# limuhit/360-Image-Compression

Measured on AMD Instinct MI355X. Metric: ERP Mpixels/s enc+dec @512x1024 model-idx 3; bitstream bit-exact vs ref, higher is better.
Workload: dtype f32; 1 GPU; 192/GPU synthetic 512x1024 ERPs, model-idx 3 --ssim seed, latent+importance bitstreams, entropy enc+dec; streams=3, masks=smooth

## Files before the change

### 360-image-compression_amd/csrc/cconv144_kernels.hip

```cpp
#include "common.h"
#include "conv_plan.h"
#include "cconv_tree.h"

#define I144_THREADS 512

template <int C, int HIDDEN>
struct ITerms {
    static constexpr int NIDX = 25 * C;
    static constexpr bool causal(int tap) { return tap / 5 + tap % 5 <= 3 + HIDDEN; }
    static constexpr int nterms(int l) {
        int n = 0;
        for (int i = l; i < NIDX; i += 128) n += causal(i % 25) ? 1 : 0;
        return n;
    }
    static constexpr int term(int l, int t) {
        int n = 0;
        for (int i = l; i < NIDX; i += 128)
            if (causal(i % 25)) { if (n == t) return i; ++n; }
        return -1;
    }
    static constexpr int nquads(int l) { return (nterms(l) + 3) / 4; }
    static constexpr int qbase(int l) {
        int s = 0;
        for (int j = 0; j < l; ++j) s += nquads(j);
        return s;
    }
    static constexpr int NQ = qbase(128);
    static constexpr int nblocks(int c) { int s = 0; for (int a = 0; a < 16; ++a) s += nquads(c + 8 * a); return s; }
    static constexpr int blk_a(int c, int b) { int a = 0; while (b >= nquads(c + 8 * a)) { b -= nquads(c + 8 * a); ++a; } return a; }
    static constexpr int blk_q(int c, int b) { int a = 0; while (b >= nquads(c + 8 * a)) { b -= nquads(c + 8 * a); ++a; } return b; }
    static constexpr int ngroups() { int m = 0; for (int c = 0; c < 8; ++c) { const int g = (nblocks(c) + 3) / 4; m = g > m ? g : m; } return m; }
    static constexpr int NG = ngroups();
};

static inline bool conv144_ok(const lic360_conv_plan *p) {
    return p->ksz == 5 && p->ngroup == 1 && p->C == 144 && p->nout >= 1 && p->nout <= 144 && p->constrain == 6;
}
template <int HIDDEN> static int i144_nq() { return ITerms<144, HIDDEN>::NQ; }
static int conv144_nq(const lic360_conv_plan *p) { (void)p; return i144_nq<1>(); }
static int conv144_otiles(const lic360_conv_plan *p) { return (p->nout + 15) / 16; }

__global__ void k_conv144_pack(const float *__restrict__ weight, const int *__restrict__ src, const int *__restrict__ qmap, float *__restrict__ packed,
                               int nout, int C, int NG, long total) {
    for (long e = (long)blockIdx.x * blockDim.x + threadIdx.x; e < total; e += (long)gridDim.x * blockDim.x) {
        const int jw = (int)(e & 3), l = (int)((e >> 2) & 63), i = l & 15, k = l >> 4;
        const long t = e >> 8;
        const int g = (int)(t % NG), c = (int)((t / NG) & 7), ot = (int)(t / (8 * NG)), o = ot * 16 + i;
        const int Q = qmap[(c * NG + g) * 4 + jw];
        const int s = Q >= 0 ? src[Q * 4 + k] : -1;
        packed[e] = (s >= 0 && o < nout) ? weight[(long)o * C * 25 + s] : 0.0f;
    }
}
template <int HIDDEN>
static void i144_fill_src(int *src, int *qmap) {
    using T = ITerms<144, HIDDEN>;
    int Q = 0;
    for (int l = 0; l < 128; ++l) {
        const int nt = T::nterms(l);
        for (int q = 0; q < T::nquads(l); ++q, ++Q)
            for (int k = 0; k < 4; ++k) src[Q * 4 + k] = 4 * q + k < nt ? T::term(l, 4 * q + k) : -1;
    }
    for (int c = 0; c < 8; ++c)
        for (int b = 0; b < 4 * T::NG; ++b)
            qmap[c * 4 * T::NG + b] = b < T::nblocks(c) ? T::qbase(c + 8 * T::blk_a(c, b)) + T::blk_q(c, b) : -1;
}
LIC360_API int lic360_conv144_supported(const lic360_conv_plan *p) { return p && conv144_ok(p) ? 1 : 0; }
LIC360_API long lic360_conv144_packed_floats(const lic360_conv_plan *p) {
    return p && conv144_ok(p) ? (long)conv144_otiles(p) * 8 * ITerms<144, 1>::NG * 256 : 0;
}
LIC360_API int lic360_conv144_pack(void *stream, const lic360_conv_plan *p, const float *weight, float *packed) {
    ARG_CHECK(p && conv144_ok(p) && weight && packed);
    const int NQ = conv144_nq(p), NG = ITerms<144, 1>::NG, nint = 4 * NQ + 8 * 4 * NG;
    std::vector<int> h(nint);
    i144_fill_src<1>(h.data(), h.data() + 4 * NQ);
    DevBuf<int> d;
    if (d.alloc(nint)) return 1;
    HIP_TRY(hipMemcpyAsync(d, h.data(), sizeof(int) * nint, hipMemcpyHostToDevice, (hipStream_t)stream));
    const long total = lic360_conv144_packed_floats(p);
    hipLaunchKernelGGL(k_conv144_pack, dim3(lic360_blocks(total, 4)), dim3(256), 0, (hipStream_t)stream, weight, d, d + 4 * NQ, packed, p->nout, p->C, NG,
                       total);
    LAUNCH_CHECK();
    HIP_TRY(hipStreamSynchronize((hipStream_t)stream));
    return 0;
}

template <bool DC, int NT>
struct ILay {
    static constexpr int ROWS = DC ? 5 : NT + 4, COLS = DC ? 16 * NT + 4 : 20, QPR = COLS / 4, PLANE = ROWS * COLS, TOFF = DC ? 16 : COLS;
    static constexpr int tap_off(int kh, int kw) { return DC ? (kh + kw) * COLS + kh : kh * COLS + kw; }
};

struct I144Args {
    const float *x, *packed, *bias, *act, *residual;
    float *out;
    int N, H, W, nout, n_ot;
    int grid;
    long xplane, xsample;
    int xpitch;
    long oplane, osample;
    int opitch, ooff;
    int tiles_r, tiles_c;
    int s, th_lo, th_hi, th0;
    int n_seg;
    int og, n_og;
};

#define I144_WAIT0() asm volatile("s_waitcnt vmcnt(0)" ::: "memory")
__device__ __forceinline__ void i144_dma_x4(const float *src, unsigned lds_byte_addr) {
    asm volatile("s_mov_b32 m0, %1\n\ts_nop 0\n\tglobal_load_lds_dwordx4 %0, off" ::"v"(src), "s"(lds_byte_addr) : "memory");
}
__device__ __forceinline__ unsigned i144_lds_addr(const float *p) {
    return (unsigned)(unsigned long)(__attribute__((address_space(3))) const float *)p;
}
__device__ __forceinline__ f32x4 i144_mfma(float a, float b, f32x4 c) { return __builtin_amdgcn_mfma_f32_16x16x4f32(a, b, c, 0, 0, 0); }

#define I144_PFG 2

template <int HIDDEN, bool DC, int NT, int WAVE>
__device__ __forceinline__ void i144_body(const I144Args &a, float *xs, float *comb, const int tid, const int lane) {
    using T = ITerms<144, HIDDEN>;
    using L = ILay<DC, NT>;
    constexpr int C = 144;
    constexpr int XQ = C * L::ROWS * L::QPR;
    constexpr int NDMA = (XQ + 511) / 512;
    const unsigned lds_x = i144_lds_addr(xs);
    int soff[NDMA];
#pragma unroll
    for (int m = 0; m < NDMA; ++m) {
        int e = (WAVE + 8 * m) * 64 + lane;
        if (e >= XQ) e = XQ - 1;
        const int pl = e / (L::ROWS * L::QPR), rem = e - pl * (L::ROWS * L::QPR), row = rem / L::QPR, cq = rem - row * L::QPR;
        soff[m] = (int)(pl * a.xplane) + row * a.xpitch + cq * 4;
    }
    const int kq = lane >> 4, j = lane & 15;
    const int ntasks = DC ? a.N * a.n_og * a.n_seg : a.N * a.tiles_r * a.tiles_c;
    int parity = 0;
    for (int task = blockIdx.x; task < ntasks; task += a.grid) {
        int n, r0 = 0, c0 = 0, ot_lo = 0, ot_hi = a.n_ot, th0 = 0;
        if constexpr (DC) {
            const int per = a.n_og * a.n_seg;
            n = task / per;
            const int rem = task - n * per, seg = rem / a.n_og;
            ot_lo = (rem - seg * a.n_og) * a.og;
            ot_hi = ot_lo + a.og < a.n_ot ? ot_lo + a.og : a.n_ot;
            th0 = a.th0 + seg * (16 * NT);
        } else {
            n = task / (a.tiles_r * a.tiles_c);
            const int rem = task - n * (a.tiles_r * a.tiles_c);
            r0 = (rem / a.tiles_c) * NT;
            c0 = (rem % a.tiles_c) * 16;
        }
        const float *xt = a.x + (long)n * a.xsample + (DC ? (long)(a.s - 4 + I144_R0) * a.xpitch + th0 : (long)r0 * a.xpitch + c0);
        __syncthreads();
        static_for<NDMA>([&](auto mm) {
            constexpr int m = decltype(mm)::value;
            if constexpr ((WAVE + 8 * m) * 64 < XQ) i144_dma_x4(xt + soff[m], lds_x + (unsigned)((WAVE + 8 * m) * 1024));
        });
        I144_WAIT0();
        __syncthreads();
        for (int ot = ot_lo; ot < ot_hi; ++ot) {
            const float *wot = a.packed + ((long)ot * 8 + WAVE) * (T::NG * 256) + lane * 4;
            f32x4 acc[NT][16];
            constexpr int NB = T::nblocks(WAVE), NGW = (NB + 3) / 4, RING = I144_PFG + 1;
            f32x4 aring[RING];
            static_for<(I144_PFG < NGW ? I144_PFG : NGW)>([&](auto gg) {
                constexpr int g = decltype(gg)::value;
                aring[g % RING] = *(const f32x4 *)(wot + g * 256);
            });
            static_for<NB>([&](auto bb) {
                constexpr int b = decltype(bb)::value, aa = T::blk_a(WAVE, b), q = T::blk_q(WAVE, b), l = WAVE + 8 * aa;
                if constexpr (b % 4 == 0 && b / 4 + I144_PFG < NGW) aring[(b / 4 + I144_PFG) % RING] = *(const f32x4 *)(wot + (b / 4 + I144_PFG) * 256);
                const float av = aring[(b / 4) % RING][b % 4];
                constexpr int nt = T::nterms(l);
                auto off_of = [](int k) constexpr {
                    const int t = 4 * q + k < nt ? 4 * q + k : nt - 1, idx = T::term(l, t), tap = idx % 25, gid = idx / 25;
                    return (gid * L::PLANE + L::tap_off(tap / 5, tap % 5)) * 4;
                };
                constexpr int o0 = off_of(0), o1 = off_of(1), o2 = off_of(2), o3 = off_of(3);
                int voff = kq == 1 ? o1 : o0;
                voff = kq == 2 ? o2 : voff;
                voff = kq == 3 ? o3 : voff;
                const float *bp = (const float *)((const char *)xs + voff) + j;
                float bv[NT];
#pragma unroll
                for (int t = 0; t < NT; ++t) bv[t] = bp[t * L::TOFF];
                __builtin_amdgcn_sched_barrier(0);
                const f32x4 zero4 = {0.f, 0.f, 0.f, 0.f};
#pragma unroll
                for (int t = 0; t < NT; ++t) acc[t][aa] = i144_mfma(av, bv[t], q == 0 ? zero4 : acc[t][aa]);
                __builtin_amdgcn_sched_barrier(0);
            });
#pragma unroll
            for (int t = 0; t < NT; ++t) {
                f32x4 lv[8];
#pragma unroll
                for (int i = 0; i < 8; ++i) lv[i] = acc[t][i] + acc[t][i + 8];
#pragma unroll
                for (int i = 0; i < 4; ++i) lv[i] = lv[i] + lv[i + 4];
#pragma unroll
                for (int i = 0; i < 2; ++i) lv[i] = lv[i] + lv[i + 2];
                const f32x4 r = lv[0] + lv[1];
#pragma unroll
                for (int v = 0; v < 4; ++v) comb[((parity * NT + t) * 8 + WAVE) * 256 + v * 64 + lane] = r[v];
            }
            __syncthreads();
            for (int e = tid; e < NT * 256; e += I144_THREADS) {
                const int t = e >> 8, rem = e & 255, v = rem >> 6, ln = rem & 63;
                const float *cb = comb + ((parity * NT + t) * 8) * 256 + v * 64 + ln;
                const float r0_ = cb[0], r1 = cb[256], r2 = cb[512], r3 = cb[768], r4 = cb[1024], r5 = cb[1280], r6 = cb[1536], r7 = cb[1792];
                float sv = ((r0_ + r4) + (r2 + r6)) + ((r1 + r5) + (r3 + r7));
                const int o = ot * 16 + 4 * (ln >> 4) + v, jj = ln & 15;
                bool ok = o < a.nout;
                long oi;
                if constexpr (DC) {
                    const int th = th0 + 16 * t + jj;
                    ok = ok && th >= a.th_lo && th <= a.th_hi;
                    oi = (long)n * a.osample + (long)o * a.oplane + (long)(a.s + I144_R0) * a.opitch + th + I144_C0;
                } else {
                    const int y = r0 + t, xx = c0 + jj;
                    ok = ok && y < a.H && xx < a.W;
                    oi = (long)n * a.osample + (long)o * a.oplane + (long)(y + a.ooff) * a.opitch + xx + a.ooff;
                }
                if (ok) {
                    sv = sv + a.bias[o];
                    if (a.act) sv = DC ? (sv < 0 ? sv * a.act[o] : sv) : (sv > 0 ? sv : sv * a.act[o]);
                    if (a.residual) sv = sv + a.residual[oi];
                    a.out[oi] = sv;
                }
            }
            parity ^= 1;
        }
    }
}

template <int HIDDEN, bool DC, int NT>
__global__ __launch_bounds__(I144_THREADS, 2) void k_cconv144(I144Args a) {
    using L = ILay<DC, NT>;
    __shared__ float xs[144 * L::PLANE + 256];
    __shared__ float comb[2 * NT * 8 * 256];
    const int tid = threadIdx.x, lane = tid & 63;
    const int wave = __builtin_amdgcn_readfirstlane(tid >> 6);
    switch (wave) {
        case 0: i144_body<HIDDEN, DC, NT, 0>(a, xs, comb, tid, lane); break;
        case 1: i144_body<HIDDEN, DC, NT, 1>(a, xs, comb, tid, lane); break;
        case 2: i144_body<HIDDEN, DC, NT, 2>(a, xs, comb, tid, lane); break;
        case 3: i144_body<HIDDEN, DC, NT, 3>(a, xs, comb, tid, lane); break;
        case 4: i144_body<HIDDEN, DC, NT, 4>(a, xs, comb, tid, lane); break;
        case 5: i144_body<HIDDEN, DC, NT, 5>(a, xs, comb, tid, lane); break;
        case 6: i144_body<HIDDEN, DC, NT, 6>(a, xs, comb, tid, lane); break;
        default: i144_body<HIDDEN, DC, NT, 7>(a, xs, comb, tid, lane); break;
    }
}

#define I144_NT_EC 2
#define I144_NT_DC 2

LIC360_API int lic360_ec144_layout(int h, int w, int *hp, int *wp) {
    ARG_CHECK(hp && wp && h > 0 && w > 0);
    *hp = (h + I144_NT_EC - 1) / I144_NT_EC * I144_NT_EC + 4;
    *wp = (w + 15) / 16 * 16 + 4;
    return 0;
}
LIC360_API int lic360_cconv144_ec(void *stream, const lic360_conv_plan *p, const float *x, const float *packed144, const float *bias,
                                  const float *act, const float *residual, float *out, int n, int h, int w, long oplane, int opitch, int ooff) {
    ARG_CHECK(p && conv144_ok(p) && x && packed144 && bias && out && n > 0 && h > 0 && w > 0 && oplane > 0 && opitch > 0 && (ooff == 0 || ooff == 2));
    I144Args a;
    int hp, wp;
    if (lic360_ec144_layout(h, w, &hp, &wp)) return 2;
    a.x = x; a.packed = packed144; a.bias = bias; a.act = act; a.residual = residual; a.out = out;
    a.N = n; a.H = h; a.W = w; a.nout = p->nout; a.n_ot = conv144_otiles(p);
    a.xplane = (long)hp * wp; a.xsample = 144 * a.xplane; a.xpitch = wp;
    a.oplane = oplane; a.osample = (long)p->nout * oplane; a.opitch = opitch; a.ooff = ooff;
    a.tiles_r = (h + I144_NT_EC - 1) / I144_NT_EC; a.tiles_c = (w + 15) / 16;
    a.s = a.th_lo = a.th_hi = a.th0 = 0; a.og = a.n_ot; a.n_og = 1; a.n_seg = 1;
    const long ntasks = (long)n * a.tiles_r * a.tiles_c;
    const dim3 grid((unsigned)(ntasks < 256 ? ntasks : 256));
    a.grid = (int)grid.x;
    hipLaunchKernelGGL((k_cconv144<1, false, I144_NT_EC>), grid, dim3(I144_THREADS), 0, (hipStream_t)stream, a);
    LAUNCH_CHECK();
    return 0;
}

LIC360_API int lic360_dc144_layout(int h, int w, int *rows, int *pitch) {
    ARG_CHECK(rows && pitch && h > 0 && w > 0);
    *rows = h + w - 1 + 2 * I144_R0;
    *pitch = (h + 2 * I144_C0 + 16 * I144_NT_DC + 3) / 4 * 4;
    return 0;
}
LIC360_API int lic360_cconv144_dc_plane(void *stream, const lic360_conv_plan *p, const float *x, const float *packed144, const float *bias,
                                        const float *act, const float *residual, float *out, int n, int h, int w, int s) {
    ARG_CHECK(p && conv144_ok(p) && x && packed144 && bias && out && n > 0 && h > 0 && w > 0);
    if (s < 0 || s >= h + w - 1) return 0;
    I144Args a;
    int rows, pitch;
    if (lic360_dc144_layout(h, w, &rows, &pitch)) return 2;
    a.x = x; a.packed = packed144; a.bias = bias; a.act = act; a.residual = residual; a.out = out;
    a.N = n; a.H = h; a.W = w; a.nout = p->nout; a.n_ot = conv144_otiles(p);
    a.xplane = (long)rows * pitch; a.xsample = 144 * a.xplane; a.xpitch = pitch;
    a.oplane = a.xplane; a.osample = (long)p->nout * a.xplane; a.opitch = pitch; a.ooff = 0;
    a.tiles_r = a.tiles_c = 1;
    a.s = s; a.th_lo = s >= w ? s - w + 1 : 0; a.th_hi = s < h ? s : h - 1; a.th0 = a.th_lo & ~3;
    a.n_seg = (a.th_hi - a.th0) / (16 * I144_NT_DC) + 1;
    a.og = a.n_ot;
    while (a.og > 1 && (long)n * a.n_seg * ((a.n_ot + a.og - 1) / a.og) < 192) --a.og;
    a.n_og = (a.n_ot + a.og - 1) / a.og;
    const long ntasks = (long)n * a.n_og * a.n_seg;
    const dim3 grid((unsigned)(ntasks < 256 ? ntasks : 256));
    a.grid = (int)grid.x;
    hipLaunchKernelGGL((k_cconv144<1, true, I144_NT_DC>), grid, dim3(I144_THREADS), 0, (hipStream_t)stream, a);
    LAUNCH_CHECK();
    return 0;
}
```

### 360-image-compression_amd/csrc/codec_fused.hip

```cpp
#include "common.h"
#include "conv_plan.h"
#include "ac_core.h"
#include "lic360_exact_math.h"
#include "gmm_tables.h"
#include "need.h"
#include <vector>
#include <cstring>
#include <algorithm>
#include <thread>
#include <atomic>
#include <memory>
#include <immintrin.h>

struct AcDevState {
    uint32_t low, high, code;
    int nacc, error, pad;
    long pos;
    unsigned long long acc;
};

struct PlanDeleter { void operator()(lic360_conv_plan *p) const { lic360_conv_plan_destroy(p); } };
using PlanPtr = std::unique_ptr<lic360_conv_plan, PlanDeleter>;
static int make_plan(PlanPtr &out, int channel, int ngroup, int nout, int ksz, int constrain) {
    lic360_conv_plan *p = nullptr;
// ... 1319 lines not shown
        return lic360_cconv144_ec(stream, nw.at(layer), xin, nw.xpack[0][layer], nw.bias[layer], nw.act[layer], res, dst, B, H, W, (long)c->e_hp * c->e_wp, c->e_wp, 2);
    };
    float *y = c->use144 ? c->e_plain : c->e_buf[1];
    if (net_walk(c->e_x0, c->use144 ? c->e_pad : c->e_buf, 3, y, ec)) return 1;
    if (c->nsym == IMP_NSYM_FAST) hipLaunchKernelGGL(k_imp_enc_tables<true>, dim3(lic360_blocks(total, 1)), dim3(64), 0, s, y, levels, c->d_pidx, c->e_rec, B, H, W, c->nsym);
    else hipLaunchKernelGGL(k_imp_enc_tables<false>, dim3(lic360_blocks(total, 1)), dim3(64), 0, s, y, levels, c->d_pidx, c->e_rec, B, H, W, c->nsym);
    LAUNCH_CHECK();
    hipLaunchKernelGGL(k_ac_encode, dim3(B), dim3(128), 0, s, c->e_rec, (long)c->HW, bytes, cap, nbytes, err);
    LAUNCH_CHECK();
    return 0;
}
struct ImpMaskPlaneArgs {
    const float *levels;
    const int *idx;
    int start;
    int len;
    float *out;
    int B;
    int H;
    int W;
    int C;
    int s;
    int cpn;
};
__global__ void k_imp_mask_plane(const ImpMaskPlaneArgs a) {
    const float *__restrict__ levels = a.levels;
    const int *__restrict__ idx = a.idx;
    const int start = a.start;
    const int len = a.len;
    float *__restrict__ out = a.out;
    const int B = a.B;
    const int H = a.H;
    const int W = a.W;
    const int C = a.C;
    const int s = a.s;
    const int cpn = a.cpn;
    const long HW = (long)H * W, total = (long)B * len * C;
    const int Co = C / (s * s), Ho = H * s, Wo = W * s;
    const long e = (long)blockIdx.x * 256 + threadIdx.x;
    if (e < total) {
        const int tc = (int)(e % C), i = (int)((e / C) % len), b = (int)(e / C / len);
        const int th = idx[start + i], tw = idx[start + i + HW];
        const int imp = (int)((double)levels[(long)b * HW + (long)th * W + tw] + 1e-5) * cpn;
        const int pc = tc / (s * s), r = tc % (s * s), ph = th * s + r / s, pw = tw * s + r % s;
        out[(((long)b * Co + pc) * Ho + ph) * Wo + pw] = tc < imp ? 1.0f : 0.0f;
    }
}
static int impcodec_decode_impl(void *stream, lic360_impcodec *c, const uint8_t *bytes, long cap, const int *nbytes, int B,
                                float *levels_out, int *err, float *mask_out, int mask_c, int stride) {
    if (check_ready(c, B)) return 2;
    ARG_CHECK(nbytes && levels_out && err);
    if (check_slot(bytes, cap)) return 2;
    hipStream_t s = (hipStream_t)stream;
    const int H = c->H, W = c->W;
    hipLaunchKernelGGL(k_dec_init, dim3((B + 63) / 64), dim3(64), 0, s, bytes, cap, nbytes, c->d_state, B);
    LAUNCH_CHECK();
    const int *pih = c->h_pidx.data();
    const long SK = (long)c->sk_rows * c->sk_pitch, off0 = (long)c->sk_row0 * c->sk_pitch + c->sk_col0;
    const NetWeights &nw = c->w;
    for (int p = 0; p < c->P; ++p) {
        if (net_walk(c->d_x0, c->d_act, 11, c->d_y, [&](int layer, const float *xin, const float *res, float *dst) -> int {
                if (c->use144 && layer > 0)
                    return lic360_cconv144_dc_plane(stream, nw.at(layer), xin, nw.xpack[0][layer], nw.bias[layer], nw.act[layer], res, dst, B, H, W, p);
                return lic360_cconv_dc_plane_strided(stream, nw.at(layer), xin + off0, nw.packed[layer], nw.bias[layer], nw.act[layer],
                                                     res ? res + off0 : nullptr, dst + off0, B, H, W, 1, c->d_idx, c->d_pidx, pih, p, B,
                                                     SK, c->sk_pitch + 1, c->sk_pitch, SK, c->sk_pitch + 1, c->sk_pitch);
            })) return 1;
        const int start = pih[p], len = pih[p + 1] - pih[p];
        if (len <= 0) continue;
        if (c->nsym == IMP_NSYM_FAST)
            hipLaunchKernelGGL(k_imp_dec_tables<true>, dim3((len + 63) / 64, B), dim3(64), 0, s, ImpDecTablesArgs{c->d_y, c->d_idx, start, len, c->d_tab, c->tab_pitch, H, W, c->nsym,
                               c->sk_rows, c->sk_pitch, c->sk_row0, c->sk_col0});
        else
            hipLaunchKernelGGL(k_imp_dec_tables<false>, dim3((len + 63) / 64, B), dim3(64), 0, s, ImpDecTablesArgs{c->d_y, c->d_idx, start, len, c->d_tab, c->tab_pitch, H, W, c->nsym,
                               c->sk_rows, c->sk_pitch, c->sk_row0, c->sk_col0});
        LAUNCH_CHECK();
        hipLaunchKernelGGL(k_imp_dec_plane<false>, dim3(B), dim3(64), 0, s, ImpDecPlaneArgs{c->d_tab, c->tab_pitch, c->d_idx, start, len, c->d_state, bytes, cap, nbytes,
                           c->d_x0, levels_out, H, W, c->nsym, c->sc, c->sk_rows, c->sk_pitch, c->sk_row0, c->sk_col0});
        LAUNCH_CHECK();
        if (mask_out) {
            const long tot = (long)B * len * mask_c;
            hipLaunchKernelGGL(k_imp_mask_plane, dim3((unsigned)((tot + 255) / 256)), dim3(256), 0, s, ImpMaskPlaneArgs{levels_out, c->d_idx, start, len, mask_out, B, H, W,
                               mask_c, stride, mask_c / (c->nsym - 1)});
            LAUNCH_CHECK();
            HIP_TRY(hipEventRecord(c->plane_ev[p], s));
        }
    }
    hipLaunchKernelGGL(k_collect_err, dim3((B + 63) / 64), dim3(64), 0, s, c->d_state, err, B);
    LAUNCH_CHECK();
    return 0;
}
LIC360_API int lic360_impcodec_decode(void *stream, lic360_impcodec *c, const uint8_t *bytes, long cap, const int *nbytes, int B,
                                      float *levels_out, int *err) {
    return impcodec_decode_impl(stream, c, bytes, cap, nbytes, B, levels_out, err, nullptr, 0, 0);
}
LIC360_API int lic360_impcodec_decode_masked(void *stream, lic360_impcodec *c, const uint8_t *bytes, long cap, const int *nbytes, int B,
                                             float *levels_out, int *err, float *mask_out, int mask_c, int stride, long *generation_out) {
    ARG_CHECK(c && mask_out && generation_out && mask_c > 0 && stride > 0 && mask_c % (stride * stride) == 0 && c->nsym > 1 &&
              mask_c % (c->nsym - 1) == 0 && B > 0 && B <= c->maxB);
    while ((int)c->plane_ev.size() < c->P) {
        HipEvent e;
        if (e.create(hipEventDisableTiming | hipEventDisableSystemFence)) return 1;
        c->plane_ev.push_back(std::move(e));
    }
    const int rc = impcodec_decode_impl(stream, c, bytes, cap, nbytes, B, levels_out, err, mask_out, mask_c, stride);
    c->gate_armed = rc == 0;
    if (rc) return rc;
    c->gate_stride = stride;
    c->gate_B = B;
    c->gate_mask = mask_out;
    *generation_out = ++c->gate_gen;
    return 0;
}

LIC360_API int lic360_codec_decode_gated(void *stream, lic360_codec *c, const uint8_t *bytes, long cap, const int *nbytes,
                                         const float *mask, int B, float *code_out, int *err, lic360_impcodec *map_codec, long generation) {
    ARG_CHECK(map_codec && generation > 0);
    if (!map_codec->gate_armed || map_codec->gate_gen != generation) {
        lic360_set_error("lic360_codec_decode_gated: stale gate (generation %ld, the map codec is at %ld, %s): enqueue "
                         "lic360_impcodec_decode_masked of THIS step first, and use each gate once",
                         generation, map_codec->gate_gen, map_codec->gate_armed ? "armed" : "already consumed");
        return 2;
    }
    if (map_codec->gate_mask != mask) {
        lic360_set_error("lic360_codec_decode_gated: `mask` is not the buffer the masked decode of generation %ld fills", generation);
        return 2;
    }
    if (B > map_codec->gate_B) {
        lic360_set_error("lic360_codec_decode_gated: batch %d, but the masked decode of generation %ld fills the mask of %d images", B, generation, map_codec->gate_B);
        return 2;
    }
    if (const int rc = check_decode(c, bytes, cap, nbytes, mask, B, code_out, err)) return rc;
    map_codec->gate_armed = false;
    return codec_decode_impl(stream, c, bytes, cap, nbytes, mask, B, code_out, err, map_codec->plane_ev.data(), map_codec->P,
                             map_codec->gate_stride);
}

__global__ void k_test_records(const int *__restrict__ tables, int ncode, const int *__restrict__ labels, const float *__restrict__ mask,
                               long n, uint2 *__restrict__ rec) {
    GRID_STRIDE(i, n) {
        uint2 r = make_uint2(0u, 0u);
        if (!mask || !(mask[i] < 0.5f)) {
            const int *T = tables + i * (ncode + 1);
            int sym = labels[i];
            sym = sym < 0 ? 0 : (sym > ncode - 1 ? ncode - 1 : sym);
            r = make_uint2((unsigned)T[sym], (unsigned)T[sym + 1]);
        }
        rec[i] = r;
    }
}
__global__ void k_test_tab8(const int *__restrict__ tables, const float *__restrict__ mask, long start, int len, uint4 *__restrict__ tab, AcDevState *st) {
    const int i = blockIdx.x * blockDim.x + threadIdx.x;
    if (i >= len) return;
    const int *T = tables + (start + i) * 9;
    const bool coded = !mask || !(mask[start + i] < 0.5f);
    if (coded && ((T[1] | T[2] | T[3] | T[4] | T[5] | T[6] | T[7]) & ~0xffff)) atomicOr(&st->error, 64);
    if (coded && T[7] == 0) atomicOr(&st->error, 64);
    uint4 r = make_uint4(0u, 0u, 0u, 0u), r2 = r;
    if (coded) dec_pack8(T, r, r2);
    tab[2 * i] = r;
    tab[2 * i + 1] = r2;
}
__global__ void k_test_tabn(const int *__restrict__ tables, int ncode, long start, int len, int *__restrict__ tab) {
    const int i = blockIdx.x, k = threadIdx.x;
    if (i < len && k <= ncode) tab[(long)i * IMP_TW + k] = tables[(start + i) * (ncode + 1) + k];
}

LIC360_API int lic360_devcoder_encode(void *stream, const int *tables, int ncode, const int *labels, const float *mask, long n,
                                      uint8_t *bytes, long cap, int *nbytes, int *err) {
    ARG_CHECK(ncode >= 1 && n >= 0 && nbytes && err && (n == 0 || (tables && labels)));
    if (check_slot(bytes, cap)) return 2;
    hipStream_t s = (hipStream_t)stream;
    DevBuf<uint2> rec;
    if (rec.alloc((size_t)n)) return 1;
    if (n) {
        hipLaunchKernelGGL(k_test_records, dim3(lic360_blocks(n, 1)), dim3(256), 0, s, tables, ncode, labels, mask, n, rec);
        LAUNCH_CHECK();
    }
    hipLaunchKernelGGL(k_ac_encode, dim3(1), dim3(128), 0, s, rec, n, bytes, cap, nbytes, err);
    LAUNCH_CHECK();
    HIP_TRY(hipStreamSynchronize(s));
    return 0;
}

LIC360_API int lic360_devcoder_decode(void *stream, const int *tables, int ncode, const float *mask, long n, int chunk,
                                      const uint8_t *bytes, long cap, const int *nbytes, float *out, int *err) {
    ARG_CHECK(ncode >= 1 && ncode < IMP_TW && n >= 0 && chunk > 0 && nbytes && out && err && (n == 0 || tables) && (ncode == 8 || !mask));
    if (check_slot(bytes, cap)) return 2;
    hipStream_t s = (hipStream_t)stream;
    DevBuf<AcDevState> st;
    DevBuf<uint4> tab8;
    DevBuf<int> tabn;
    if (st.alloc(1) || tab8.alloc(2 * (size_t)chunk) || tabn.alloc((size_t)chunk * IMP_TW)) return 1;
    hipLaunchKernelGGL(k_dec_init, dim3(1), dim3(64), 0, s, bytes, cap, nbytes, st, 1);
    LAUNCH_CHECK();
    for (long start = 0; start < n; start += chunk) {
        const int len = (int)std::min<long>(chunk, n - start);
        if (ncode == 8) {
            hipLaunchKernelGGL(k_test_tab8, dim3((len + 63) / 64), dim3(64), 0, s, tables, mask, start, len, tab8, st);
            LAUNCH_CHECK();
            hipLaunchKernelGGL(k_dec_plane<true>, dim3(1), dim3(64), 0, s, DecPlaneArgs{tab8, chunk, (const int *)nullptr, (int)start, len, 0, st, bytes, cap, nbytes,
                               (float *)nullptr, out, 0, 1, 1, 0, 0, 0, 0});
        } else {
            hipLaunchKernelGGL(k_test_tabn, dim3(len), dim3(64), 0, s, tables, ncode, start, len, tabn);
            LAUNCH_CHECK();
            hipLaunchKernelGGL(k_imp_dec_plane<true>, dim3(1), dim3(64), 0, s, ImpDecPlaneArgs{tabn, chunk, (const int *)nullptr, (int)start, len, st, bytes, cap, nbytes,
                               (float *)nullptr, out, 0, 0, ncode, 0.0f});
        }
        LAUNCH_CHECK();
    }
    hipLaunchKernelGGL(k_collect_err, dim3(1), dim3(64), 0, s, st, err, 1);
    LAUNCH_CHECK();
    HIP_TRY(hipStreamSynchronize(s));
    return 0;
}

LIC360_API int lic360_codec_profile_enable(lic360_codec *c, int on) {
    ARG_CHECK(c);
    c->prof = on != 0;
    for (int k = 0; k < PROF_NCLS; ++k) c->n_ev[k] = 0;
    return 0;
}
LIC360_API const char *lic360_codec_profile_classes(void) { return PROF_NAMES; }

LIC360_API int lic360_codec_profile_read(lic360_codec *c, int n, double *ms, long *launches) {
    ARG_CHECK(c && ms && launches && n >= PROF_NCLS);
    for (int k = 0; k < PROF_NCLS; ++k) {
        double acc = 0;
        const size_t cnt = c->n_ev[k];
        for (size_t i = 0; i + 1 < cnt; i += 2) {
            HIP_TRY(hipEventSynchronize(c->ev[k][i + 1]));
            float t = 0;
            HIP_TRY(hipEventElapsedTime(&t, c->ev[k][i], c->ev[k][i + 1]));
            acc += t;
        }
        ms[k] = acc;
        launches[k] = (long)(cnt / 2);
        c->n_ev[k] = 0;
    }
    return 0;
}

LIC360_API int lic360_codec_skip_stats(lic360_codec *c, int enable, unsigned long long *out, int *skip_active_out) {
    ARG_CHECK(c);
    if (skip_active_out) *skip_active_out = c->skip ? 1 + (c->dcl.list ? 1 : 0) : 0;
    if (!c->skip) { if (out) memset(out, 0, 2 * NEED_LAYERS * NEED_STAT_G * sizeof(unsigned long long)); return 0; }
    if (enable >= 0) c->stats_on = enable != 0;
    if (out) {
        HIP_TRY(hipDeviceSynchronize());
        HIP_TRY(hipMemcpy(out, c->stats, 2 * NEED_LAYERS * NEED_STAT_G * sizeof(unsigned long long), hipMemcpyDeviceToHost));
        HIP_TRY(hipMemset(c->stats, 0, 2 * NEED_LAYERS * NEED_STAT_G * sizeof(unsigned long long)));
    }
    return 0;
}
__global__ void k_fill_enc(float *buf, long planes, int H, int W, int hp, int wp, int off, float v) {
    GRID_STRIDE(i, planes * H * W) {
        const int x = (int)(i % W), y = (int)((i / W) % H);
        buf[(i / ((long)H * W)) * hp * wp + e_cell(y, x, wp, off)] = v;
    }
}
__global__ void k_fill_dec(float *buf, long planes, int H, int W, int sk_rows, int sk_pitch, int row0, int col0, float v) {
    GRID_STRIDE(i, planes * H * W) {
        const int x = (int)(i % W), y = (int)((i / W) % H);
        buf[(i / ((long)H * W)) * sk_rows * sk_pitch + (long)(y + x + row0) * sk_pitch + y + col0] = v;
    }
}
LIC360_API int lic360_codec_debug_fill(void *stream, lic360_codec *c, float value) {
    ARG_CHECK(c && value == value && value - value == 0.0f);
    hipStream_t s = (hipStream_t)stream;
    const long B = c->maxB, G = c->G;
    for (int i = 0; i < 3; ++i) {
        hipLaunchKernelGGL(k_fill_enc, dim3(lic360_blocks(3 * B * 4 * G * c->HW, 4)), dim3(256), 0, s, c->e_buf[i], 3 * B * 4 * G, c->H, c->W, c->e_hp, c->e_wp, c->e_off, value);
        LAUNCH_CHECK();
    }
    for (int i = 0; i < 11; ++i) {
        hipLaunchKernelGGL(k_fill_dec, dim3(lic360_blocks(3 * B * 4 * G * c->HW, 4)), dim3(256), 0, s, c->d_act[i], 3 * B * 4 * G, c->H, c->W, c->sk_rows, c->sk_pitch, c->sk_row0, c->sk_col0, value);
        LAUNCH_CHECK();
    }
    hipLaunchKernelGGL(k_fill_dec, dim3(lic360_blocks(3 * B * 3 * G * c->HW, 4)), dim3(256), 0, s, c->d_y, 3 * B * 3 * G, c->H, c->W, c->sk_rows, c->sk_pitch, c->sk_row0, c->sk_col0, value);
    LAUNCH_CHECK();
    return 0;
}
LIC360_API int lic360_codec_debug_lists(lic360_codec *c, int which, void *host_out, long bytes, int *cap_out) {
    ARG_CHECK(c && host_out && bytes >= 0 && which >= 0 && which <= 4 && c->skip);
    HIP_TRY(hipDeviceSynchronize());
    const void *src = nullptr;
    long have = 0;
    if (which == 0) { src = c->need; have = (long)c->maxB * NEED_LAYERS * c->HW; }
    else if (which == 1) { src = c->ecl.cnt; have = NEED_LAYERS * 8 * 4L; }
    else if (which == 2) { src = c->ecl.list; have = (long)NEED_LAYERS * 8 * c->ecl.cap * 4; }
    else if (which == 3) { src = c->dcl.cnt; have = c->dcl.list ? (long)NEED_LAYERS * c->P * 8 * 4 : 0; }
    else { src = c->dcl.list; have = c->dcl.list ? (long)NEED_LAYERS * c->P * 8 * c->dcl.cap * 16 : 0; }
    if (cap_out) *cap_out = which <= 2 ? c->ecl.cap : c->dcl.cap;
    ARG_CHECK(src && bytes <= have);
    HIP_TRY(hipMemcpy(host_out, src, (size_t)bytes, hipMemcpyDeviceToHost));
    return 0;
}

LIC360_API const char *lic360_codec_kernel_names(void) {
    return "ec_first=k_cconv16<1, false>;ec_hidden=k_cconv16s+k_cconv16<4, false>;ec_last=k_cconv16<4, true>;"
           "dc_first=k_cconv4v6<1, false, false>+k_cconv4v6t<1>;"
           "dc_hidden=k_cconv4v6l<4>+k_cconv4v6t<4>+k_cconv4v6<4, false, false>+k_cconv4v6<4, false, true>;"
           "dc_last=k_cconv4v6l<4>+k_cconv4v6t<4>+k_cconv4v6<4, false, false>+k_cconv4v6<4, false, true>;"
           "imp_ec=k_cconv144<1, false, 2>;imp_dc=k_cconv144<1, true, 2>";
}
```

Before: 59.52 Mpixel/s.

## Pipeline LDS B-operand reads and weight prefetch across output tiles in cconv144

Software-pipelines the LDS reads of the B operand BD blocks ahead of the MFMAs through a register ring. The weight-ring prefetch for the next output tile is now issued before the epilogue, and the first one overlaps the input DMA. The epilogue is reassigned to one cell per thread, with its bias, activation and residual loads hoisted ahead of the MFMA loop. A new NT=1 instantiation is launched for short decode diagonals that fit in a single 16-wide segment, which avoids wasted tile work. These changes raise register pressure and code size, which could lower occupancy.

Result: faster. 60.14 Mpixel/s, median of 6 (+1.0%).

```diff
diff --git a/360-image-compression_amd/csrc/cconv144_kernels.hip b/360-image-compression_amd/csrc/cconv144_kernels.hip
--- a/360-image-compression_amd/csrc/cconv144_kernels.hip
+++ b/360-image-compression_amd/csrc/cconv144_kernels.hip
@@ -115,6 +115,12 @@
 __device__ __forceinline__ f32x4 i144_mfma(float a, float b, f32x4 c) { return __builtin_amdgcn_mfma_f32_16x16x4f32(a, b, c, 0, 0, 0); }
 
 #define I144_PFG 2
+#ifndef I144_BD
+#define I144_BD 2
+#endif
+#ifndef I144_BAS
+#define I144_BAS 5
+#endif
 
 template <int HIDDEN, bool DC, int NT, int WAVE>
 __device__ __forceinline__ void i144_body(const I144Args &a, float *xs, float *comb, const int tid, const int lane) {
@@ -156,40 +162,74 @@
             constexpr int m = decltype(mm)::value;
             if constexpr ((WAVE + 8 * m) * 64 < XQ) i144_dma_x4(xt + soff[m], lds_x + (unsigned)((WAVE + 8 * m) * 1024));
         });
+        constexpr int NB = T::nblocks(WAVE), NGW = (NB + 3) / 4, PFG = I144_PFG * 2 / NT, RING = PFG + 1;
+        f32x4 aring[RING];
+        const float *wot = a.packed + ((long)ot_lo * 8 + WAVE) * (T::NG * 256) + lane * 4;
+        auto a_head = [&]() {
+            static_for<(PFG < NGW ? PFG : NGW)>([&](auto gg) {
+                constexpr int g = decltype(gg)::value;
+                aring[g % RING] = *(const f32x4 *)(wot + g * 256);
+            });
+        };
+        a_head();
         I144_WAIT0();
         __syncthreads();
         for (int ot = ot_lo; ot < ot_hi; ++ot) {
-            const float *wot = a.packed + ((long)ot * 8 + WAVE) * (T::NG * 256) + lane * 4;
+            static_assert(NT * 256 <= I144_THREADS, "one epilogue cell per thread");
+            constexpr bool EPI = WAVE * 64 < NT * 256;
+            const int e_t = WAVE >> 2, e_v = WAVE & 3, e_o = ot * 16 + 4 * kq + e_v;
+            bool e_ok = EPI && e_o < a.nout;
+            long e_oi;
+            if constexpr (DC) {
+                const int th = th0 + 16 * e_t + j;
+                e_ok = e_ok && th >= a.th_lo && th <= a.th_hi;
+                e_oi = (long)n * a.osample + (long)e_o * a.oplane + (long)(a.s + I144_R0) * a.opitch + th + I144_C0;
+            } else {
+                const int y = r0 + e_t, xx = c0 + j;
+                e_ok = e_ok && y < a.H && xx < a.W;
+                e_oi = (long)n * a.osample + (long)e_o * a.oplane + (long)(y + a.ooff) * a.opitch + xx + a.ooff;
+            }
+            float e_bias = 0.f, e_act = 0.f, e_res = 0.f;
+            if (e_ok) {
+                e_bias = a.bias[e_o];
+                if (a.act) e_act = a.act[e_o];
+                if (a.residual) e_res = a.residual[e_oi];
+            }
             f32x4 acc[NT][16];
-            constexpr int NB = T::nblocks(WAVE), NGW = (NB + 3) / 4, RING = I144_PFG + 1;
-            f32x4 aring[RING];
-            static_for<(I144_PFG < NGW ? I144_PFG : NGW)>([&](auto gg) {
-                constexpr int g = decltype(gg)::value;
-                aring[g % RING] = *(const f32x4 *)(wot + g * 256);
-            });
-            static_for<NB>([&](auto bb) {
+            constexpr int BD = I144_BD * 2 / NT, BRING = BD + 1;
+            float bring[BRING][NT];
+            int kq_ot = kq;
+            asm volatile("" : "+v"(kq_ot));
+            auto b_read = [&](auto bb) {
                 constexpr int b = decltype(bb)::value, aa = T::blk_a(WAVE, b), q = T::blk_q(WAVE, b), l = WAVE + 8 * aa;
-                if constexpr (b % 4 == 0 && b / 4 + I144_PFG < NGW) aring[(b / 4 + I144_PFG) % RING] = *(const f32x4 *)(wot + (b / 4 + I144_PFG) * 256);
-                const float av = aring[(b / 4) % RING][b % 4];
                 constexpr int nt = T::nterms(l);
                 auto off_of = [](int k) constexpr {
                     const int t = 4 * q + k < nt ? 4 * q + k : nt - 1, idx = T::term(l, t), tap = idx % 25, gid = idx / 25;
                     return (gid * L::PLANE + L::tap_off(tap / 5, tap % 5)) * 4;
                 };
                 constexpr int o0 = off_of(0), o1 = off_of(1), o2 = off_of(2), o3 = off_of(3);
-                int voff = kq == 1 ? o1 : o0;
-                voff = kq == 2 ? o2 : voff;
-                voff = kq == 3 ? o3 : voff;
+                const int kqb = NT > 1 && b % I144_BAS == I144_BAS - 1 ? kq_ot : kq;
+                int voff = kqb == 1 ? o1 : o0;
+                voff = kqb == 2 ? o2 : voff;
+                voff = kqb == 3 ? o3 : voff;
                 const float *bp = (const float *)((const char *)xs + voff) + j;
-                float bv[NT];
-#pragma unroll
-                for (int t = 0; t < NT; ++t) bv[t] = bp[t * L::TOFF];
+#pragma unroll
+                for (int t = 0; t < NT; ++t) bring[b % BRING][t] = bp[t * L::TOFF];
+            };
+            static_for<(BD < NB ? BD : NB)>(b_read);
+            static_for<NB>([&](auto bb) {
+                constexpr int b = decltype(bb)::value, aa = T::blk_a(WAVE, b), q = T::blk_q(WAVE, b);
+                if constexpr (b % 4 == 0 && b / 4 + PFG < NGW) aring[(b / 4 + PFG) % RING] = *(const f32x4 *)(wot + (b / 4 + PFG) * 256);
+                const float av = aring[(b / 4) % RING][b % 4];
+                if constexpr (b + BD < NB) b_read(IC<b + BD>{});
                 __builtin_amdgcn_sched_barrier(0);
                 const f32x4 zero4 = {0.f, 0.f, 0.f, 0.f};
 #pragma unroll
-                for (int t = 0; t < NT; ++t) acc[t][aa] = i144_mfma(av, bv[t], q == 0 ? zero4 : acc[t][aa]);
+                for (int t = 0; t < NT; ++t) acc[t][aa] = i144_mfma(av, bring[b % BRING][t], q == 0 ? zero4 : acc[t][aa]);
                 __builtin_amdgcn_sched_barrier(0);
             });
+            wot += 8 * (T::NG * 256);
+            if (ot + 1 < ot_hi) a_head();
 #pragma unroll
             for (int t = 0; t < NT; ++t) {
                 f32x4 lv[8];
@@ -204,28 +244,15 @@
                 for (int v = 0; v < 4; ++v) comb[((parity * NT + t) * 8 + WAVE) * 256 + v * 64 + lane] = r[v];
             }
             __syncthreads();
-            for (int e = tid; e < NT * 256; e += I144_THREADS) {
-                const int t = e >> 8, rem = e & 255, v = rem >> 6, ln = rem & 63;
-                const float *cb = comb + ((parity * NT + t) * 8) * 256 + v * 64 + ln;
+            if constexpr (EPI) {
+                const float *cb = comb + ((parity * NT + e_t) * 8) * 256 + e_v * 64 + lane;
                 const float r0_ = cb[0], r1 = cb[256], r2 = cb[512], r3 = cb[768], r4 = cb[1024], r5 = cb[1280], r6 = cb[1536], r7 = cb[1792];
                 float sv = ((r0_ + r4) + (r2 + r6)) + ((r1 + r5) + (r3 + r7));
-                const int o = ot * 16 + 4 * (ln >> 4) + v, jj = ln & 15;
-                bool ok = o < a.nout;
-                long oi;
-                if constexpr (DC) {
-                    const int th = th0 + 16 * t + jj;
-                    ok = ok && th >= a.th_lo && th <= a.th_hi;
-                    oi = (long)n * a.osample + (long)o * a.oplane + (long)(a.s + I144_R0) * a.opitch + th + I144_C0;
-                } else {
-                    const int y = r0 + t, xx = c0 + jj;
-                    ok = ok && y < a.H && xx < a.W;
-                    oi = (long)n * a.osample + (long)o * a.oplane + (long)(y + a.ooff) * a.opitch + xx + a.ooff;
-                }
-                if (ok) {
-                    sv = sv + a.bias[o];
-                    if (a.act) sv = DC ? (sv < 0 ? sv * a.act[o] : sv) : (sv > 0 ? sv : sv * a.act[o]);
-                    if (a.residual) sv = sv + a.residual[oi];
-                    a.out[oi] = sv;
+                if (e_ok) {
+                    sv = sv + e_bias;
+                    if (a.act) sv = DC ? (sv < 0 ? sv * e_act : sv) : (sv > 0 ? sv : sv * e_act);
+                    if (a.residual) sv = sv + e_res;
+                    a.out[e_oi] = sv;
                 }
             }
             parity ^= 1;
@@ -307,7 +334,10 @@
     const long ntasks = (long)n * a.n_og * a.n_seg;
     const dim3 grid((unsigned)(ntasks < 256 ? ntasks : 256));
     a.grid = (int)grid.x;
-    hipLaunchKernelGGL((k_cconv144<1, true, I144_NT_DC>), grid, dim3(I144_THREADS), 0, (hipStream_t)stream, a);
+    if (a.n_seg == 1 && a.th_hi - a.th0 < 16)
+        hipLaunchKernelGGL((k_cconv144<1, true, 1>), grid, dim3(I144_THREADS), 0, (hipStream_t)stream, a);
+    else
+        hipLaunchKernelGGL((k_cconv144<1, true, I144_NT_DC>), grid, dim3(I144_THREADS), 0, (hipStream_t)stream, a);
     LAUNCH_CHECK();
     return 0;
 }
diff --git a/360-image-compression_amd/csrc/codec_fused.hip b/360-image-compression_amd/csrc/codec_fused.hip
--- a/360-image-compression_amd/csrc/codec_fused.hip
+++ b/360-image-compression_amd/csrc/codec_fused.hip
@@ -1645,5 +1645,5 @@
            "dc_first=k_cconv4v6<1, false, false>+k_cconv4v6t<1>;"
            "dc_hidden=k_cconv4v6l<4>+k_cconv4v6t<4>+k_cconv4v6<4, false, false>+k_cconv4v6<4, false, true>;"
            "dc_last=k_cconv4v6l<4>+k_cconv4v6t<4>+k_cconv4v6<4, false, false>+k_cconv4v6<4, false, true>;"
-           "imp_ec=k_cconv144<1, false, 2>;imp_dc=k_cconv144<1, true, 2>";
-}
+           "imp_ec=k_cconv144<1, false, 2>;imp_dc=k_cconv144<1, true, 2>+k_cconv144<1, true, 1>";
+}
```
